# Gadersd/stable-diffusion-burn

Hardware: NVIDIA H100
Metric: images_per_sec_512x512_20steps (higher is better)
Workload: dtype fp16 tensor-core operands (3-term split-fp16 on the two high-res UNet levels), fp32 accumulate

## Files before the change

### include/sdb200.h

```cpp
#ifndef SDB200_H
#define SDB200_H

#include <stddef.h>
#include <stdint.h>

#ifdef __cplusplus
extern "C" {
#endif

typedef struct sdb_ctx sdb_ctx;

int sdb_create(int device, sdb_ctx** out);
int sdb_create_inpaint(int device, sdb_ctx** out);
int sdb_destroy(sdb_ctx* ctx);
const char* sdb_last_error(sdb_ctx* ctx);
const char* sdb_version(void);

int sdb_tensor_count(sdb_ctx* ctx);
int sdb_tensor_info(sdb_ctx* ctx, int index, const char** name, int64_t dims[4], int* ndim);
int sdb_set_tensor(sdb_ctx* ctx, const char* name, const float* host, const int64_t* dims, int ndim);
int sdb_get_tensor(sdb_ctx* ctx, const char* name, float* host, int64_t count);
int sdb_load_dump_dir(sdb_ctx* ctx, const char* path);
int64_t sdb_read_dump_tensor(const char* file, int ndim, int64_t* dims, float* data, int64_t capacity);
int sdb_init_synthetic(sdb_ctx* ctx, uint32_t seed);
// ... 76 lines not shown
int sdb_profile_get(sdb_ctx* ctx, int cls, const char** name, int64_t* launches, double* ms,
                    double* flops, double* bytes);
int sdb_profile_get_issued(sdb_ctx* ctx, int cls, double* issued_flops);
int64_t sdb_launch_count(sdb_ctx* ctx);

int sdb_test_linear(sdb_ctx* ctx, const float* a, const float* w, const float* bias, int M, int K, int N,
                    int passes, float* c);
int sdb_test_gemm_ex(sdb_ctx* ctx, const float* a, const float* w, const float* bias, const float* residual, int M, int K,
                     int N, int passes, int flags, const float* xa, const float* xw, int XK, float* out);
int sdb_test_conv2d(sdb_ctx* ctx, const float* x, const float* w, const float* bias, int n, int cin, int H,
                    int W, int cout, int ksize, int stride, int upsample, int passes, float* y);
int sdb_test_ln_fold(sdb_ctx* ctx, const float* a, const float* a2, const float* w0, const float* b0, const float* gamma,
                     const float* beta, const float* w1, const float* b1, int M, int K0, int C, int N, int passes, int geglu,
                     float* out);
int sdb_test_conv_groupnorm(sdb_ctx* ctx, const float* x, const float* w, const float* bias, const float* gamma,
                            const float* beta, int n, int cin, int H, int W, int cout, int ksize, int stride, int upsample,
                            int passes, int silu, float* y, int* slots);
int sdb_test_groupnorm(sdb_ctx* ctx, const float* x, const float* gamma, const float* beta, int n, int c,
                       int H, int W, int silu, float* y);
int sdb_test_layernorm(sdb_ctx* ctx, const float* x, const float* gamma, const float* beta, int rows, int c,
                       float* y);
int sdb_test_attention(sdb_ctx* ctx, const float* q, const float* k, const float* v, int n, int Nq, int Nk,
                       int C, int heads, const int32_t* kvlen, int flags, float* out);
int sdb_test_resblock(sdb_ctx* ctx, const float* x0, const float* x1, int n, int c0, int c1, int H, int W, int cout,
                      const float* norm1_g, const float* norm1_b, const float* conv1_w, const float* conv1_b, const float* norm2_g,
                      const float* norm2_b, const float* conv2_w, const float* conv2_b, const float* skip_w, const float* skip_b,
                      const float* emb_bias, int passes, int flags, float* out, float* out16, float* out_norm, int32_t* trace);
int sdb_test_groupnorm_cat(sdb_ctx* ctx, const float* x0, const float* x1, int n, int c0, int c1, int H, int W,
                           const float* gamma, const float* beta, int silu, int mode, float* y, int32_t* trace);
int sdb_test_spatial_transformer(sdb_ctx* ctx, int index, const float* x, int n, int c, int H, int W, const float* context,
                                 int lmax, const int32_t* lens, int flags, float* out, float* out16, float* out_norm, float* taps_y,
                                 float* taps_ln, int32_t* trace);
int sdb_test_step_noise(sdb_ctx* ctx, uint64_t noise_seed, int t, int64_t count, float* out);

#ifdef __cplusplus
}
#endif
#endif
```

### stable_diffusion_burn_b200/_lib.py

```python
from __future__ import annotations

import ctypes as C
import os

import numpy as np

_HERE = os.path.dirname(os.path.abspath(__file__))
LIB_PATH = os.path.join(_HERE, "libsdb200.so")

_f32p = C.POINTER(C.c_float)
_u8p = C.POINTER(C.c_uint8)
_i64p = C.POINTER(C.c_int64)
_ctx = C.c_void_p


class SdbBatch(C.Structure):
    _fields_ = [("n", C.c_int), ("L", C.c_int), ("context", C.c_void_p), ("context_len", C.POINTER(C.c_int32)),
                ("Lu", C.c_int), ("uncond", C.c_void_p), ("uncond_len", C.POINTER(C.c_int32)),
                ("guidance_scale", C.POINTER(C.c_double)), ("seed", C.POINTER(C.c_uint64)),
                ("noise_seed", C.POINTER(C.c_uint64))]


_batchp = C.POINTER(SdbBatch)

# ... 46 lines not shown
    ("sdb_lora_remove", C.c_int, [_ctx, C.c_int]),
    ("sdb_lora_apply", C.c_int, [_ctx]),
    ("sdb_get_merged_tensor", C.c_int, [_ctx, C.c_char_p, _f32p, C.c_int64]),
    ("sdb_sample_batch", C.c_int, [_ctx, _batchp, C.c_int, _f32p, C.c_int, C.c_int, _f32p, _u8p]),
    ("sdb_sample_batch_dev", C.c_int, [_ctx, _batchp, C.c_int, C.c_void_p, C.c_int, C.c_int, C.c_void_p, C.c_void_p,
                                       C.c_void_p]),
    ("sdb_img2img_batch", C.c_int, [_ctx, _batchp, _u8p, _u8p, C.c_double, C.c_int, _f32p, C.c_int, C.c_int, _f32p, _u8p]),
    ("sdb_img2img_batch_dev", C.c_int, [_ctx, _batchp, C.c_void_p, C.c_void_p, C.c_double, C.c_int, C.c_void_p, C.c_int,
                                        C.c_int, C.c_void_p, C.c_void_p, C.c_void_p]),
    ("sdb_set_option", C.c_int, [_ctx, C.c_char_p, C.c_int]),
    ("sdb_profile_enable", C.c_int, [_ctx, C.c_int]),
    ("sdb_profile_reset", C.c_int, [_ctx]),
    ("sdb_profile_class_count", C.c_int, [_ctx]),
    ("sdb_profile_get", C.c_int, [_ctx, C.c_int, C.POINTER(C.c_char_p), _i64p, C.POINTER(C.c_double),
                                  C.POINTER(C.c_double), C.POINTER(C.c_double)]),
    ("sdb_profile_get_issued", C.c_int, [_ctx, C.c_int, C.POINTER(C.c_double)]),
    ("sdb_launch_count", C.c_int64, [_ctx]),
    ("sdb_test_linear", C.c_int, [_ctx, _f32p, _f32p, _f32p, C.c_int, C.c_int, C.c_int, C.c_int, _f32p]),
    ("sdb_test_conv2d", C.c_int, [_ctx, _f32p, _f32p, _f32p, C.c_int, C.c_int, C.c_int, C.c_int, C.c_int, C.c_int,
                                  C.c_int, C.c_int, C.c_int, _f32p]),
    ("sdb_test_ln_fold", C.c_int, [_ctx, _f32p, _f32p, _f32p, _f32p, _f32p, _f32p, _f32p, _f32p, C.c_int, C.c_int, C.c_int, C.c_int,
                                   C.c_int, C.c_int, _f32p]),
    ("sdb_test_conv_groupnorm", C.c_int, [_ctx, _f32p, _f32p, _f32p, _f32p, _f32p, C.c_int, C.c_int, C.c_int, C.c_int, C.c_int,
                                          C.c_int, C.c_int, C.c_int, C.c_int, C.c_int, _f32p, C.POINTER(C.c_int)]),
    ("sdb_test_resblock", C.c_int, [_ctx, _f32p, _f32p, C.c_int, C.c_int, C.c_int, C.c_int, C.c_int, C.c_int,
                                    _f32p, _f32p, _f32p, _f32p, _f32p, _f32p, _f32p, _f32p, _f32p, _f32p, _f32p,
                                    C.c_int, C.c_int, _f32p, _f32p, _f32p, C.POINTER(C.c_int32)]),
    ("sdb_test_groupnorm_cat", C.c_int, [_ctx, _f32p, _f32p, C.c_int, C.c_int, C.c_int, C.c_int, C.c_int, _f32p, _f32p,
                                         C.c_int, C.c_int, _f32p, C.POINTER(C.c_int32)]),
    ("sdb_test_spatial_transformer", C.c_int, [_ctx, C.c_int, _f32p, C.c_int, C.c_int, C.c_int, C.c_int, _f32p, C.c_int,
                                               C.POINTER(C.c_int32), C.c_int, _f32p, _f32p, _f32p, _f32p, _f32p,
                                               C.POINTER(C.c_int32)]),
    ("sdb_test_step_noise", C.c_int, [_ctx, C.c_uint64, C.c_int, C.c_int64, _f32p]),
    ("sdb_test_groupnorm", C.c_int, [_ctx, _f32p, _f32p, _f32p, C.c_int, C.c_int, C.c_int, C.c_int, C.c_int, _f32p]),
    ("sdb_test_layernorm", C.c_int, [_ctx, _f32p, _f32p, _f32p, C.c_int, C.c_int, _f32p]),
    ("sdb_test_attention", C.c_int, [_ctx, _f32p, _f32p, _f32p, C.c_int, C.c_int, C.c_int, C.c_int, C.c_int,
                                     C.POINTER(C.c_int32), C.c_int, _f32p]),
]

_lib = None


def load():
    global _lib
    if _lib is None:
        if not os.path.exists(LIB_PATH):
            raise RuntimeError(f"{LIB_PATH} is missing: build it with `python -c 'import __graft_entry__ as g; g.build()'` "
                               "(there is no CPU fallback)")
        lib = C.CDLL(LIB_PATH)
        for name, res, args in SIGNATURES:
            fn = getattr(lib, name)
            fn.restype = res
            fn.argtypes = args
        _lib = lib
    return _lib


def f32(a) -> np.ndarray:
    return np.ascontiguousarray(a, dtype=np.float32)


def ptr(a: np.ndarray):
    return a.ctypes.data_as(_f32p)


class SdbError(RuntimeError):
# ... 436 lines not shown
    def test_groupnorm_cat(self, x0, x1, gamma, beta, silu=False, mode=0):
        x0 = f32(x0)
        n, c0, H, W = x0.shape
        x1 = f32(x1) if x1 is not None else None
        c1 = 0 if x1 is None else x1.shape[1]
        g = f32(gamma); b = f32(beta)
        y = np.empty((n, c0 + c1, H, W), np.float32)
        trace = np.zeros(64, np.int32)
        self.check(self.lib.sdb_test_groupnorm_cat(self.h, ptr(x0), None if x1 is None else ptr(x1), n, c0, c1, H, W, ptr(g), ptr(b),
                                                   1 if silu else 0, int(mode), ptr(y), trace.ctypes.data_as(C.POINTER(C.c_int32))))
        return y, self._decode_trace(trace)

    _EPI_ROLES = ("lns", "lnc", "geglu", "res16", "res32", "gn")

    def test_spatial_transformer(self, index, x, context, lens, act16=True):
        x = f32(x); context = f32(context)
        n, c, H, W = x.shape
        lens = np.ascontiguousarray(lens, dtype=np.int32)
        assert context.shape[0] == n and context.shape[2] == 768 and lens.shape == (n,)
        out, out16, outn = (np.empty((n, c, H, W), np.float32) for _ in range(3))
        y = np.empty((4, n * H * W, c), np.float32)
        ln = np.empty((3, n * H * W, 2), np.float32)
        t = np.zeros(160, np.int32)
        i32 = lambda a: a.ctypes.data_as(C.POINTER(C.c_int32))
        self.check(self.lib.sdb_test_spatial_transformer(self.h, int(index), ptr(x), n, c, H, W, ptr(context), context.shape[1],
                                                         i32(lens), 1 if act16 else 0, ptr(out), ptr(out16), ptr(outn), ptr(y),
                                                         ptr(ln), i32(t)))
        paths = {1: "fused", 2: "apply", 3: "apply+fold"}
        keys = ("kind", "N", "BN", "split", "TN", "TH", "TW", "xk", "gn_slots", "a1", "passes")
        gemms = []
        for i in range(min(int(t[5]), 10)):
            g = dict(zip(keys, (int(v) for v in t[6 + 12 * i:17 + 12 * i])))
            g["epi"] = {r for b, r in enumerate(self._EPI_ROLES) if int(t[17 + 12 * i]) >> b & 1}
            gemms.append(g)
        attn = [dict(zip(("dpad", "Nq", "Nk", "qk3", "kvlen"), (int(v) for v in t[127 + 5 * i:132 + 5 * i])))
                for i in range(min(int(t[126]), 4))]
        tr = {"gn": [paths.get(int(v), int(v)) for v in t[1:1 + min(int(t[0]), 4)]], "gemms": gemms, "attn": attn}
        return dict(out=out, out16=out16, out_norm=outn, y=y, ln=ln, trace=tr)

    def test_groupnorm(self, x, gamma, beta, silu=False):
        x = f32(x); n, c, H, W = x.shape
        y = np.empty_like(x)
        g = f32(gamma); b = f32(beta)
        self.check(self.lib.sdb_test_groupnorm(self.h, ptr(x), ptr(g), ptr(b), n, c, H, W, 1 if silu else 0, ptr(y)))
        return y

    def test_step_noise(self, noise_seed, t, count):
        out = np.empty(int(count), np.float32)
        self.check(self.lib.sdb_test_step_noise(self.h, int(noise_seed), int(t), int(count), ptr(out)))
        return out

    def test_layernorm(self, x, gamma, beta):
        x = f32(x); rows, c = x.shape
        y = np.empty_like(x)
        g = f32(gamma); b = f32(beta)
        self.check(self.lib.sdb_test_layernorm(self.h, ptr(x), ptr(g), ptr(b), rows, c, ptr(y)))
        return y

    def test_attention(self, q, k, v, heads, kvlen=None, causal=False, v_transposed=False):
        q = f32(q); k = f32(k); v = f32(v)
        n, Nq, Cc = q.shape; Nk = k.shape[1]
        out = np.empty_like(q)
        lens = None if kvlen is None else np.ascontiguousarray(kvlen, dtype=np.int32)
        assert lens is None or lens.shape == (n,), "kvlen needs one length per sample"
        flags = (1 if causal else 0) | (2 if v_transposed else 0)
        self.check(self.lib.sdb_test_attention(self.h, ptr(q), ptr(k), ptr(v), n, Nq, Nk, Cc, heads,
# ... 4 lines not shown
```

### stable_diffusion_burn_b200/csrc/api.cu

```cuda
#include "../../include/sdb200.h"

#include <dlfcn.h>

#include <cstdlib>
#include <cstring>
#include <mutex>

#include "attention.cuh"
#include "kernels.cuh"
#include "model.cuh"
#include "runtime.cuh"

using namespace sdb;

struct sdb_ctx {
  Ctx c;
};

static thread_local std::string g_err;

#define API_BEGIN(ctxp)                      \
  if (!(ctxp)) {                             \
    g_err = "null context";                  \
    return 1;                                \
  }                                          \
  Ctx& c = (ctxp)->c;                        \
  try {                                      \
    SDB_CUDA(cudaSetDevice(c.device));

#define API_END                              \
  }                                          \
  catch (const std::exception& e) {          \
    c.err = e.what();                        \
    g_err = c.err;                           \
    return 1;                                \
  }                                          \
  return 0;

static void ctx_teardown(sdb_ctx* h) {
  if (!h) return;
  cudaSetDevice(h->c.device);
// ... 864 lines not shown
                      skip_w, skip_b, emb_bias, passes, flags, out, out16, out_norm, trace);
  API_END
}

int sdb_test_groupnorm_cat(sdb_ctx* ctx, const float* x0, const float* x1, int n, int c0, int c1, int H, int W, const float* gamma,
                           const float* beta, int silu, int mode, float* y, int32_t* trace) {
  API_BEGIN(ctx)
  c.work.reset();
  model_test_groupnorm_cat(c, x0, x1, n, c0, c1, H, W, gamma, beta, silu, mode, y, trace);
  API_END
}

int sdb_test_spatial_transformer(sdb_ctx* ctx, int index, const float* x, int n, int ch, int H, int W, const float* context,
                                 int lmax, const int32_t* lens, int flags, float* out, float* out16, float* out_norm, float* taps_y,
                                 float* taps_ln, int32_t* trace) {
  API_BEGIN(ctx)
  need_final(c);
  c.work.reset();
  model_test_spatial_transformer(c, index, x, n, ch, H, W, context, lmax, lens, flags, out, out16, out_norm, taps_y, taps_ln, trace);
  API_END
}

int sdb_test_step_noise(sdb_ctx* ctx, uint64_t noise_seed, int t, int64_t count, float* out) {
  API_BEGIN(ctx)
  SDB_CHECK(out && count >= 1, "step_noise: null output or count < 1");
  SDB_CHECK(t >= 0 && t < 1000, "step_noise: timestep must be in [0, 1000)");
  float* d = (float*)c.io(0, (size_t)count * 4);
  step_noise_launch(d, (long long)count, noise_seed, t, c.stream);
  SDB_CUDA(cudaMemcpyAsync(out, d, (size_t)count * 4, cudaMemcpyDeviceToHost, c.stream));
  SDB_CUDA(cudaStreamSynchronize(c.stream));
  API_END
}

}
```

### stable_diffusion_burn_b200/csrc/model.cu

```cuda
#include "model.cuh"

#include "../../include/sdb200.h"

#include <algorithm>
#include <cmath>
#include <cstring>
#include <functional>

#include "model_def.cuh"

namespace sdb {

static Model& M(Ctx& c) { return *reinterpret_cast<Model*>(c.model); }
static int round_up(int x, int m) { return (x + m - 1) / m * m; }

static int g_level_passes[4] = {3, 3, 1, 1};
static int g_vae_passes_lowres = 3, g_vae_passes_up = 3, g_vae_passes_highres = 1;

static Half2Ptr alloc_half2(Arena& a, size_t count) {
  Half2Ptr p;
  p.hi = a.get<__half>(count);
  p.lo = a.get<__half>(count);
  return p;
}
// ... 2186 lines not shown
  SpatialTransformerW& st = *m.sts[index];
  SDB_CHECK(Cx == st.c, "test_spatial_transformer: x must have the block's channel count (" + std::to_string(st.c) + ")");
  const int C = st.c, HW = H * W, ls = ln_slots(C);
  const long long Mt = (long long)n * HW;
  Fwd f(c, n);
  f.init_sums(4);
  const int Lpad = round_up(Lmax, 32);
  float* ctxp = c.work.get<float>((size_t)n * Lpad * 768);
  int* d_len = c.work.get<int>(n);
  SDB_CUDA(cudaMemsetAsync(ctxp, 0, (size_t)n * Lpad * 768 * 4, c.stream));
  SDB_CUDA(cudaMemcpy2DAsync(ctxp, (size_t)Lpad * 768 * 4, context, (size_t)Lmax * 768 * 4, (size_t)Lmax * 768 * 4, n,
                             cudaMemcpyHostToDevice, c.stream));
  SDB_CUDA(cudaMemcpyAsync(d_len, lens, 4 * n, cudaMemcpyHostToDevice, c.stream));
  CtxState cs;
  prepare_context(f, ctxp, Lpad, d_len, cs);
  const Act a = stage_activation(f, x, C, H, W, true);
  Act o = (flags & 1) ? f.act16(H, W, C) : f.act(H, W, C);
  StTaps taps;
  for (Half2Ptr& y : taps.y) y = f.half2((size_t)Mt * C, true);
  for (float*& l : taps.ln) l = c.work.get<float>((size_t)Mt * ls * 2);
  ActOp g;
  {
    TraceScope ts(c);
    run_spatial_transformer(f, st, cs, cs.kv[index], a, o, &taps);
    g = f.gn_operand(o, nullptr, st.norm, true, true);
    std::fill(trace, trace + kStTraceInts, 0);
    trace[0] = (int)c.gn_trace.size();
    for (size_t i = 0; i < c.gn_trace.size() && i < 4; ++i) trace[1 + i] = c.gn_trace[i];
    trace[5] = (int)c.gemm_trace.size();
    for (size_t i = 0; i < c.gemm_trace.size() && i < 10; ++i) {
      const Ctx::GemmRecord& r = c.gemm_trace[i];
      const int v[12] = {r.kind, r.N, r.BN, r.split, r.TN, r.TH, r.TW, r.xk_channels, r.gn_slots, r.a1_channels, r.passes, r.epi};
      std::copy(v, v + 12, trace + 6 + 12 * i);
    }
    trace[126] = (int)c.attn_trace.size();
    for (size_t i = 0; i < c.attn_trace.size() && i < 4; ++i) {
      const Ctx::AttnRecord& r = c.attn_trace[i];
      const int v[5] = {r.dpad, r.Nq, r.Nk, r.qk3, r.kvlen};
      std::copy(v, v + 5, trace + 127 + 5 * i);
    }
  }
  float* d = c.work.get<float>(o.count());
  nhwc_to_nchw_launch(o.p, n, C, H, W, d, c.stream);
  SDB_CUDA(cudaMemcpyAsync(out, d, o.count() * 4, cudaMemcpyDeviceToHost, c.stream));
  fetch_half2(c, o.raw16, n, C, H, W, out16);
  fetch_half2(c, g.p, n, C, H, W, out_norm);
  const size_t cnt = (size_t)Mt * C;
  std::vector<__half> hi(cnt), lo(cnt);
  for (int i = 0; i < 4; ++i) {
    SDB_CUDA(cudaMemcpyAsync(hi.data(), taps.y[i].hi, cnt * 2, cudaMemcpyDeviceToHost, c.stream));
    SDB_CUDA(cudaMemcpyAsync(lo.data(), taps.y[i].lo, cnt * 2, cudaMemcpyDeviceToHost, c.stream));
    SDB_CUDA(cudaStreamSynchronize(c.stream));
    for (size_t e = 0; e < cnt; ++e) taps_y[i * cnt + e] = __half2float(hi[e]) + __half2float(lo[e]);
  }
  std::vector<float> sl((size_t)Mt * ls * 2);
  for (int i = 0; i < 3; ++i) {
    SDB_CUDA(cudaMemcpyAsync(sl.data(), taps.ln[i], sl.size() * 4, cudaMemcpyDeviceToHost, c.stream));
    SDB_CUDA(cudaStreamSynchronize(c.stream));
    for (long long r = 0; r < Mt; ++r) {
      float sm = 0.f, sq = 0.f;
      for (int k = 0; k < ls; ++k) sm += sl[(r * ls + k) * 2], sq += sl[(r * ls + k) * 2 + 1];
      taps_ln[(i * Mt + r) * 2] = sm, taps_ln[(i * Mt + r) * 2 + 1] = sq;
    }
  }
}

// ... 2 lines not shown
```

### stable_diffusion_burn_b200/csrc/runtime.cu

```cuda
#include "runtime.cuh"

#include <algorithm>

#include <cudaTypedefs.h>

#include <cmath>
#include <cstdlib>
#include <cstring>

namespace sdb {

int g_pdl_late = 1;
bool g_pdl_enabled = true;
int g_num_sms = 132;

void Arena::init(size_t bytes) {
  SDB_CUDA(cudaMalloc(&base, bytes));
  cap = bytes;
  off = 0;
}
void Arena::destroy() {
  if (base) cudaFree(base);
  base = nullptr;
  cap = off = 0;
}
void* Arena::alloc(size_t bytes) {
  const size_t a = (off + 1023) & ~size_t(1023);
  if (a + bytes > cap)
    throw Error("arena exhausted: need " + std::to_string(a + bytes) + " of " + std::to_string(cap) + " bytes");
  off = a + bytes;
  if (off > high) high = off;
  return base + a;
}
// ... 268 lines not shown
    SDB_CHECK(xk->x0.n == a0.n && xk->x0.H == a0.H && xk->x0.W == a0.W && xk->x0.P == 1 && xk->x0.C % 64 == 0, "extra-K geometry");
    SDB_CHECK(!xk->has_x1 || (xk->x1.n == a0.n && xk->x1.H == a0.H && xk->x1.W == a0.W && xk->x1.C % 64 == 0), "extra-K geometry");
    SDB_CHECK(xk->w.N == w.N && xk->w.K == xC, "extra-K weights");
    SDB_CHECK(passes < 2 || (xk->x0.p.lo && (!xk->has_x1 || xk->x1.p.lo)), "multi-pass GEMM needs the lo half of the extra operands");
    SDB_CHECK(passes < 3 || xk->w.p.lo, "3-pass GEMM needs the lo half of the extra weights");
    p.xkc0 = xk->x0.C / 64, p.xkc = xC / 64;
  }

  p.TW = std::min(pow2_floor(a0.W), 128);
  p.TH = std::min(128 / p.TW, pow2_ceil(a0.H));
  p.TN = 128 / (p.TW * p.TH);
  p.tiles_w = (a0.W + p.TW - 1) / p.TW;
  p.tiles_h = (a0.H + p.TH - 1) / p.TH;
  p.tiles_n = (a0.n + p.TN - 1) / p.TN;
  const int m_tiles = p.tiles_w * p.tiles_h * p.tiles_n;

  int BN;
  if (ep.geglu)
    BN = 128;
  else if (w.N % 160 == 0)
    BN = 160;
  else if (w.N % 256 == 0 && (long long)m_tiles * (w.N / 256) >= 2 * g_num_sms)
    BN = 256;
  else if (w.N % 128 == 0)
    BN = 128;
  else
    BN = 64;
  if (ep.ln_out) {
    SDB_CHECK(w.N % 160 == 0 && !ep.geglu, "LayerNorm statistics need an output width that tiles by 160");
    BN = 160;
  }
  if (ep.ln_in) SDB_CHECK(BN == 128 || BN == 160, "LayerNorm-consuming GEMM: tile width");
  const int n_tiles = (w.N + BN - 1) / BN;


  const int iters = p.num_taps * p.kc + p.xkc;
  int split = 1;
  if (c.opt_splitk && kind != G_CONV3_UP2 && !ep.geglu && !ep.ln_out && !ep.ln_in) {
    const int ctas = m_tiles * n_tiles;
    if (ctas <= g_num_sms / 2 && iters >= c.opt_splitk_min_iters) {
      split = std::min(std::min(g_num_sms / ctas, iters / c.opt_splitk_chunk), 16);
      if (split < 1) split = 1;
    }
  }
  if (split > 1) {
    const int per = (iters + split - 1) / split;
    split = (iters + per - 1) / per;
  }
  p.split_k = split;
  static const bool gemm_dbg = getenv("SDB_GEMM_DBG") != nullptr || getenv("SDB_LABEL_LOG") != nullptr;
  if (c.debug_sync || c.profiling || gemm_dbg) {
    char buf[256];
    snprintf(buf, sizeof(buf), "gemm kind=%d n=%d H=%d W=%d P=%d C0=%d C1=%d N=%d K=%d xk=%d BN=%d split=%d passes=%d geglu=%d epi=%s%s tile=%dx%dx%d",
             kind, a0.n, a0.H, a0.W, a0.P, a0.C, a1in ? a1.C : 0, w.N, w.K, p.xkc * 64, BN, split, passes, ep.geglu,
             ep.gn ? "gn" : (ep.ln_out ? "lns" : (ep.ln_in ? "lnc" : "-")), ep.residual16.hi ? "+r16" : (ep.residual ? "+r32" : ""), p.TN, p.TH, p.TW);
    c.dbg_label = buf;
  }

  GnPart* gn = ep.gn;
  if (gn) {
    int slots = m_tiles / p.tiles_n * split * phases_out;
    bool geom = p.TN <= 4;
    if (kind == G_LINEAR && gn_rpi > 0) {
      const long long rows = (long long)a0.W;
      geom = rows % gn_rpi == 0 && (gn_rpi % 128 == 0 || (128 % gn_rpi == 0 && gn_rpi >= 32));
      gn_nimg = (int)(rows / gn_rpi);
      slots = (gn_rpi >= 128 ? gn_rpi / 128 : 1) * split;
    } else {
      if (kind == G_LINEAR) geom = false;
      gn_rpi = 0;
    }
    const bool ok = gn->buf && gn->bucket > 0 && !ep.geglu && geom && BN >= 128 && BN % gn->bucket == 0 && w.N % gn->bucket == 0 &&
                    slots <= gn->cap && c.opt_gn_epilogue;
    gn->slots = ok ? slots : 0;
    if (!ok) gn = nullptr;
  }
  if (c.trace_on) {
    const int epi = (ep.ln_out ? EPI_ROLE_LNS : 0) | (ep.ln_in ? EPI_ROLE_LNC : 0) | (ep.geglu ? EPI_ROLE_GEGLU : 0) |
                    (ep.residual16.hi ? EPI_ROLE_RES16 : 0) | (ep.residual ? EPI_ROLE_RES32 : 0) | (gn ? EPI_ROLE_GN : 0);
    c.gemm_trace.push_back({kind_in, w.N, BN, split, p.TN, p.TH, p.TW, p.xkc * 64, gn ? gn->slots : 0, a1in ? a1.C : 0, passes, epi});
  }
  p.gn_part = gn ? gn->buf : nullptr;
  p.gn_cap = gn ? gn->cap : 0, p.gn_bucket = gn ? gn->bucket : 1;
  p.gn_rpi = gn ? gn_rpi : 0, p.gn_nimg = gn_nimg;
  p.ln_out = ep.ln_out, p.ln_slots = ln_slots(w.N);
  p.ln_in = ep.ln_in, p.ln_in_slots = ep.ln_in_slots, p.ln_C = ep.ln_C, p.ln_eps = ep.ln_eps;
  p.ln_u = passes >= 3 ? ep.ln_u_full : ep.ln_u_hi;
  SDB_CHECK(!ep.ln_in || (p.ln_u && ep.ln_in_slots > 0 && ep.ln_C == w.K && kind == G_LINEAR), "LayerNorm-consuming GEMM: arguments");
  SDB_CHECK(!ep.ln_in || (!ep.residual && !ep.rowbias && !ep.residual16.hi), "LayerNorm-consuming GEMM: no residual / row bias");
  SDB_CHECK(!ep.ln_out || kind == G_LINEAR, "LayerNorm statistics: rows must be tokens");
  p.res_hi = ep.residual16.hi, p.res_lo = ep.residual16.lo;
  SDB_CHECK(!ep.residual16.hi || (ep.residual16.lo && !ep.residual && !ep.rowbias), "fp16-pair residual: needs both halves, excludes the fp32 residual / row bias");
  p.out_f32 = ep.out_f32;
  p.out_f16 = ep.out_f16.hi;
  p.out_f16_lo = ep.out_f16.lo;
  p.bias = ep.bias;
  p.rowbias = ep.rowbias;
  p.residual = ep.residual;
  p.geglu = ep.geglu;
  p.act = ep.act;
  p.pdl_late = g_pdl_late;
  p.prefetch_w = (g_pdl_enabled && c.opt_prefetch_w && m_tiles <= 4) ? 1 : 0;
  const int nout = ep.geglu ? w.N / 2 : w.N;
  p.ldc = ep.ldc ? ep.ldc : nout;
  p.ldc16 = ep.ldc16 ? ep.ldc16 : nout;
  SDB_CHECK(!(ep.rowbias && ep.residual), "epilogue takes a time-embedding row or a residual, not both");
  p.os = (kind == G_CONV3_UP2) ? 2 : 1;
  p.OH = a0.H * p.os, p.OW = a0.W * p.os;
  SDB_CHECK((double)a0.n * p.OH * p.OW * (double)std::max(p.ldc, p.ldc16) < 2147483648.0,
            "GEMM output exceeds 2^31 elements (the epilogue uses 32-bit element offsets)");

  GemmMaps maps;
  memset(&maps, 0, sizeof(maps));
// ... 36 lines not shown
    maps.b[1] = maps.b[0];
    if (passes >= 3) maps.b[1] = make_w_map(wlo, w.K, wrows, bbox, w.ld);
    maps.bx[0] = maps.bx[1] = maps.b[0];
    if (xk) {
      const int xrows = xk->w.rows ? xk->w.rows : xk->w.N;
      maps.bx[0] = make_w_map(xk->w.p.hi, xk->w.K, xrows, bbox, xk->w.ld);
      maps.bx[1] = passes >= 3 ? make_w_map(xk->w.p.lo, xk->w.K, xrows, bbox, xk->w.ld) : maps.bx[0];
    }
    p.gn_slot0 = 0;
    p.up2 = 0, p.gn_phase_slots = (m_tiles / p.tiles_n) * split;
    if (kind == G_CONV3_UP2) {
      p.up2 = 1, p.oa = 0, p.ob = 0;
      for (int t = 0; t < 4; ++t) p.tap_dh[t] = (t >> 1) - 1, p.tap_dw[t] = (t & 1) - 1, p.tap_ph[t] = 0;
    }
    if (split > 1) {
      const size_t need = (size_t)split * (size_t)Mtot * w.N * sizeof(float);
      p.ws = reinterpret_cast<float*>(c.work.alloc(need));
      SDB_CHECK((long long)m_tiles * n_tiles * 2 <= 65536, "split-K ticket buffer");
      SDB_CHECK((long long)m_tiles * n_tiles * split <= g_num_sms, "split-K CTAs must be co-resident");
      p.tickets = c.splitk_tickets;
    }
    {
      static const bool dbg_on = getenv("SDB_GEMM_DBG") != nullptr;
      static long long* dbg_buf = nullptr;
      if (dbg_on) {
        if (!dbg_buf) SDB_CUDA(cudaMallocManaged(&dbg_buf, 16 * sizeof(long long)));
        SDB_CUDA(cudaStreamSynchronize(c.stream));
        memset(dbg_buf, 0, 16 * sizeof(long long));
        p.dbg = dbg_buf;
      }
      const std::string label = c.dbg_label;
      {
        KernelScope ks(c, KC_GEMM, flops * phases_out, bytes * phases_out, flops * passes * phases_out);
        gemm_tc_launch(maps, p, BN, passes, c.stream);
      }
      if (dbg_on) {
        SDB_CUDA(cudaStreamSynchronize(c.stream));
        fprintf(stderr, "gemm_dbg %s | cycles since entry: prologue %lld tma0 %lld landed %lld lastmma %lld accum %lld epi %lld exit %lld | chunk0: ld %lld stage %lld finish %lld (bias %lld loads0 %lld batch0 %lld)\n",
                label.c_str(), dbg_buf[1] - dbg_buf[0], dbg_buf[2] - dbg_buf[0], dbg_buf[3] - dbg_buf[0],
                dbg_buf[4] - dbg_buf[0], dbg_buf[5] - dbg_buf[0], dbg_buf[6] - dbg_buf[0], dbg_buf[7] - dbg_buf[0], dbg_buf[9] - dbg_buf[8], dbg_buf[10] - dbg_buf[9],
                dbg_buf[11] - dbg_buf[10], dbg_buf[12] - dbg_buf[10], dbg_buf[13] - dbg_buf[12], dbg_buf[14] - dbg_buf[13]);
      }
    }
  }
}

}
```

### stable_diffusion_burn_b200/csrc/runtime.cuh

```cuda
#pragma once
#include <string>
#include <unordered_map>
#include <unordered_set>
#include <vector>

#include "common.cuh"
#include "attention.cuh"
#include "gemm_tc.cuh"
#include "kernels.cuh"

namespace sdb {

struct Arena {
  char* base = nullptr;
  size_t cap = 0, off = 0, high = 0;
  void init(size_t bytes);
  void destroy();
  void* alloc(size_t bytes);
  template <class T>
  T* get(size_t count) {
    return reinterpret_cast<T*>(alloc(count * sizeof(T)));
  }
  void reset() { off = 0; }
};
// ... 95 lines not shown
  std::unordered_map<std::string, float> norm_eps;
  int opt_precision = 0;
  int opt_graphs = 1;
  int opt_splitk = 1;
  int opt_splitk_min_iters = 32, opt_splitk_chunk = 8;
  int opt_skip_merge = 1;
  int opt_raw16 = 1;
  int opt_mlp_passes = 0;
  int opt_attn_split = 1;
  int opt_emb_hoist = 1;
  int opt_prefetch_w = 0;
  int opt_gn_epilogue = 1;
  int sampler_kind = 0;
  double sampler_eta = 0.0;
  uint64_t sampler_noise_seed = 0;
  int unet_cin = 4;
  bool profiling = false;
  std::vector<ProfEvent> prof;
  int64_t launches = 0;
  double cls_ms[KC_COUNT] = {0}, cls_flops[KC_COUNT] = {0}, cls_bytes[KC_COUNT] = {0};
  double cls_issued[KC_COUNT] = {0};
  int64_t cls_launches[KC_COUNT] = {0};
  struct IoBuf {
    void* p = nullptr;
    size_t cap = 0;
  } iobuf[13];
  void* io(int slot, size_t bytes);
  void io_destroy();
  void* model = nullptr;
  unsigned int* splitk_tickets = nullptr;
  bool debug_sync = false;
  std::string dbg_label;
  struct GemmRecord {
    int kind, N, BN, split, TN, TH, TW, xk_channels, gn_slots, a1_channels, passes, epi;
  };
  struct AttnRecord {
    int dpad, Nq, Nk, qk3, kvlen;
  };
  bool trace_on = false;
  std::vector<GemmRecord> gemm_trace;
  std::vector<AttnRecord> attn_trace;
  std::vector<int> gn_trace;

  float* master_ptr(const std::string& name);
  const TensorInfo& info(const std::string& name);
  bool has(const std::string& name) const { return index.count(name) != 0; }
};

struct KernelScope {
  Ctx& c;
  int cls;
  bool on;
  ProfEvent ev;
  KernelScope(Ctx& c, int cls, double flops = 0, double bytes = 0, double issued = 0);
  ~KernelScope();
};
void profile_collect(Ctx& c);

struct ExtraK {
  ActOp x0, x1;
  bool has_x1 = false;
  WeightOp w;
};

void run_gemm(Ctx& c, int kind, const ActOp& a0, const ActOp* a1, const WeightOp& w, int passes, const Epilogue& ep,
              const ExtraK* xk = nullptr);

// ... 23 lines not shown
```

Before: 5.000.

## Add persistent warp-specialized GEGLU GEMM with LayerNorm-consuming epilogue

Adds a persistent TMA+wgmma kernel for the LayerNorm-consuming GEGLU GEMM with 3-pass split-fp16 operands. It is selected when the tile count exceeds the SM count. A producer warp streams A/B chunks through a multi-stage mbarrier ring while two consumer warpgroups alternate tiles, so one group's epilogue overlaps the other's MMA. This is meant to remove wave-quantization and per-tile prologue/epilogue stalls, at the cost of a fixed BN=128 constraint and a new code path that needs its own correctness checks. It also adds a host schedule API and a trace flag for testing.

```diff
diff --git a/include/sdb200.h b/include/sdb200.h
--- a/include/sdb200.h
+++ b/include/sdb200.h
@@ -132,6 +132,7 @@
                                  int lmax, const int32_t* lens, int flags, float* out, float* out16, float* out_norm, float* taps_y,
                                  float* taps_ln, int32_t* trace);
 int sdb_test_step_noise(sdb_ctx* ctx, uint64_t noise_seed, int t, int64_t count, float* out);
+int sdb_gemm_lnc_schedule(int ntiles, int kchunks, int num_sms, int stages, int32_t* out);
 
 #ifdef __cplusplus
 }
diff --git a/stable_diffusion_burn_b200/_lib.py b/stable_diffusion_burn_b200/_lib.py
--- a/stable_diffusion_burn_b200/_lib.py
+++ b/stable_diffusion_burn_b200/_lib.py
@@ -102,6 +102,7 @@
                                                C.POINTER(C.c_int32), C.c_int, _f32p, _f32p, _f32p, _f32p, _f32p,
                                                C.POINTER(C.c_int32)]),
     ("sdb_test_step_noise", C.c_int, [_ctx, C.c_uint64, C.c_int, C.c_int64, _f32p]),
+    ("sdb_gemm_lnc_schedule", C.c_int, [C.c_int, C.c_int, C.c_int, C.c_int, C.POINTER(C.c_int32)]),
     ("sdb_test_groupnorm", C.c_int, [_ctx, _f32p, _f32p, _f32p, C.c_int, C.c_int, C.c_int, C.c_int, C.c_int, _f32p]),
     ("sdb_test_layernorm", C.c_int, [_ctx, _f32p, _f32p, _f32p, C.c_int, C.c_int, _f32p]),
     ("sdb_test_attention", C.c_int, [_ctx, _f32p, _f32p, _f32p, C.c_int, C.c_int, C.c_int, C.c_int, C.c_int,
@@ -604,6 +605,7 @@
         for i in range(min(int(t[5]), 10)):
             g = dict(zip(keys, (int(v) for v in t[6 + 12 * i:17 + 12 * i])))
             g["epi"] = {r for b, r in enumerate(self._EPI_ROLES) if int(t[17 + 12 * i]) >> b & 1}
+            g["persistent"] = bool(int(t[147]) >> i & 1)
             gemms.append(g)
         attn = [dict(zip(("dpad", "Nq", "Nk", "qk3", "kvlen"), (int(v) for v in t[127 + 5 * i:132 + 5 * i])))
                 for i in range(min(int(t[126]), 4))]
diff --git a/stable_diffusion_burn_b200/csrc/api.cu b/stable_diffusion_burn_b200/csrc/api.cu
--- a/stable_diffusion_burn_b200/csrc/api.cu
+++ b/stable_diffusion_burn_b200/csrc/api.cu
@@ -2,11 +2,13 @@
 
 #include <dlfcn.h>
 
+#include <algorithm>
 #include <cstdlib>
 #include <cstring>
 #include <mutex>
 
 #include "attention.cuh"
+#include "gemm_lnc.cuh"
 #include "kernels.cuh"
 #include "model.cuh"
 #include "runtime.cuh"
@@ -937,4 +939,18 @@
   API_END
 }
 
-}
+int sdb_gemm_lnc_schedule(int ntiles, int kchunks, int num_sms, int stages, int32_t* out) {
+  if (ntiles < 1 || kchunks < 1 || num_sms < 1 || stages < 1 || !out) return -1;
+  const int grid = std::min(ntiles, num_sms);
+  for (int cta = 0; cta < grid; ++cta) {
+    const int nseq = sdb::lnc_cta_tiles(ntiles, cta, grid) * kchunks;
+    for (int seq = 0; seq < nseq; ++seq, out += 7) {
+      const sdb::LncChunk c = sdb::lnc_chunk(seq, kchunks, cta, grid, stages);
+      const int32_t rec[7] = {cta, seq, c.tile, c.k, c.stage, (int32_t)c.phase, c.consumer};
+      std::copy(rec, rec + 7, out);
+    }
+  }
+  return 0;
+}
+
+}
diff --git a/stable_diffusion_burn_b200/csrc/gemm_lnc.cu b/stable_diffusion_burn_b200/csrc/gemm_lnc.cu
--- /dev/null
+++ b/stable_diffusion_burn_b200/csrc/gemm_lnc.cu
@@ -0,0 +1,237 @@
+#include "gemm_lnc.cuh"
+
+#include <algorithm>
+
+namespace sdb {
+
+namespace {
+
+constexpr int BM = 128;
+constexpr int BK = 64;
+constexpr int A_TILE_BYTES = BM * BK * 2;
+constexpr int SMEM_OPTIN_MAX = 227 * 1024;
+
+template <int BN>
+struct LncStage {
+  static constexpr int B_TILE_BYTES = BN * BK * 2;
+  static constexpr int BYTES = 2 * A_TILE_BYTES + 2 * B_TILE_BYTES;
+};
+template <int BN>
+__host__ __device__ constexpr int lnc_stages() {
+  constexpr int n = (SMEM_OPTIN_MAX - 1024) / (LncStage<BN>::BYTES + 2 * 8);
+  return n > 8 ? 8 : n;
+}
+
+__device__ __forceinline__ void store_pair16(float y0, float y1, unsigned int o16, __half* out_f16, __half* out_f16_lo) {
+  const __half2 h = f2h2_sat(y0, y1);
+  *reinterpret_cast<__half2*>(out_f16 + o16) = h;
+  if (out_f16_lo) {
+    const float2 f = __half22float2(h);
+    *reinterpret_cast<__half2*>(out_f16_lo + o16) = __floats2half2_rn(y0 - f.x, y1 - f.y);
+  }
+}
+
+template <int BN>
+__global__ void __launch_bounds__(384, 1)
+gemm_lnc_persistent_kernel(const __grid_constant__ GemmMaps maps, const GemmParams p, int n_tiles, int ntiles) {
+  using L = LncStage<BN>;
+  constexpr int STAGES = lnc_stages<BN>();
+  extern __shared__ __align__(1024) uint8_t smem_raw[];
+  uint8_t* smem = smem_raw + ((1024u - (smem_u32(smem_raw) & 1023u)) & 1023u);
+  uint64_t* full_bar = reinterpret_cast<uint64_t*>(smem + STAGES * L::BYTES);
+  uint64_t* empty_bar = full_bar + STAGES;
+
+  const int warp = threadIdx.x >> 5;
+  const int lane = threadIdx.x & 31;
+  const int kc = p.kc;
+  const int my_tiles = lnc_cta_tiles(ntiles, blockIdx.x, gridDim.x);
+  const int nseq = my_tiles * kc;
+  long long* const dbg = (p.dbg && blockIdx.x == 0) ? p.dbg : nullptr;
+  if (dbg && threadIdx.x == 0) dbg[0] = clock64();
+  if (!p.pdl_late) pdl_trigger();
+
+  if (threadIdx.x == 0) {
+    for (int s = 0; s < STAGES; ++s) {
+      mbar_init(&full_bar[s], 1);
+      mbar_init(&empty_bar[s], 4);
+    }
+    fence_mbar_init();
+  }
+  if (warp == 0 && lane == 0) {
+    tma_prefetch_desc(&maps.a[0][0]);
+    tma_prefetch_desc(&maps.b[0]);
+  }
+  __syncthreads();
+  if (dbg && threadIdx.x == 0) dbg[1] = clock64();
+
+  if (warp < 4) {
+    asm volatile("setmaxnreg.dec.sync.aligned.u32 40;");
+    if (warp == 0 && elect_one()) {
+      auto load_b = [&](const LncChunk& c) {
+        uint8_t* sb = smem + c.stage * L::BYTES + 2 * A_TILE_BYTES;
+        const int col0 = (c.tile % n_tiles) * BN;
+        tma_load_2d(sb, &maps.b[0], &full_bar[c.stage], c.k * BK, col0);
+        tma_load_2d(sb + L::B_TILE_BYTES, &maps.b[1], &full_bar[c.stage], c.k * BK, col0);
+      };
+      auto load_a = [&](const LncChunk& c) {
+        uint8_t* st = smem + c.stage * L::BYTES;
+        const int w0 = (c.tile / n_tiles) * BM;
+        tma_load_5d(st, &maps.a[0][0], &full_bar[c.stage], c.k * BK, w0, 0, 0, 0);
+        tma_load_5d(st + A_TILE_BYTES, &maps.a[0][1], &full_bar[c.stage], c.k * BK, w0, 0, 0, 0);
+      };
+      const int npre = min(STAGES, nseq);
+      for (int seq = 0; seq < npre; ++seq) {
+        const LncChunk c = lnc_chunk(seq, kc, blockIdx.x, gridDim.x, STAGES);
+        mbar_expect_tx(&full_bar[c.stage], L::BYTES);
+        load_b(c);
+      }
+      pdl_wait();
+      for (int seq = 0; seq < npre; ++seq) load_a(lnc_chunk(seq, kc, blockIdx.x, gridDim.x, STAGES));
+      if (dbg) dbg[2] = clock64();
+      for (int seq = npre; seq < nseq; ++seq) {
+        const LncChunk c = lnc_chunk(seq, kc, blockIdx.x, gridDim.x, STAGES);
+        mbar_wait(&empty_bar[c.stage], c.phase ^ 1u);
+        mbar_expect_tx(&full_bar[c.stage], L::BYTES);
+        load_a(c);
+        load_b(c);
+      }
+    }
+  } else {
+    asm volatile("setmaxnreg.inc.sync.aligned.u32 232;");
+    pdl_wait();
+    const int g = (warp - 4) >> 2;
+    const int wq = warp & 3;
+    const bool stamp = dbg && wq == 0 && lane == 0;
+    const int cq = 2 * (lane & 3);
+    for (int i = g; i < my_tiles; i += 2) {
+      const int tile = blockIdx.x + i * gridDim.x;
+      const int mt = tile / n_tiles, nt = tile - mt * n_tiles;
+      const bool last = i == my_tiles - 1;
+      float acc[2][BN / 2];
+#pragma unroll
+      for (int h = 0; h < 2; ++h)
+#pragma unroll
+        for (int j = 0; j < BN / 2; ++j) acc[h][j] = 0.f;
+      int prev = -1;
+      if (i > 0) asm volatile("bar.sync %0, 256;" ::"r"(1 + g) : "memory");
+      for (int k = 0; k < kc; ++k) {
+        const LncChunk c = lnc_chunk(i * kc + k, kc, blockIdx.x, gridDim.x, STAGES);
+        mbar_wait(&full_bar[c.stage], c.phase);
+        if (dbg && threadIdx.x == 128 && i == 0 && k == 0) dbg[3] = clock64();
+        const uint32_t a_hi = smem_u32(smem + c.stage * L::BYTES);
+        const uint32_t a_lo = a_hi + A_TILE_BYTES;
+        const uint32_t b_hi = a_hi + 2 * A_TILE_BYTES;
+        const uint32_t b_lo = b_hi + L::B_TILE_BYTES;
+        wgmma_fence();
+#pragma unroll
+        for (int kk = 0; kk < BK / 16; ++kk) {
+          const uint32_t koff = kk * 32;
+          const uint64_t db = make_sdesc_sw128(b_hi + koff), db_lo = make_sdesc_sw128(b_lo + koff);
+#pragma unroll
+          for (int h = 0; h < 2; ++h) {
+            const uint64_t da = make_sdesc_sw128(a_hi + h * (64 * 128) + koff);
+            Wgmma<BN>::template ss<0>(acc[h], da, db, 1);
+            Wgmma<BN>::template ss<0>(acc[h], make_sdesc_sw128(a_lo + h * (64 * 128) + koff), db, 1);
+            Wgmma<BN>::template ss<0>(acc[h], da, db_lo, 1);
+          }
+        }
+        wgmma_commit();
+        wgmma_wait<1>();
+        if (prev >= 0 && lane == 0) mbar_arrive(&empty_bar[prev]);
+        prev = c.stage;
+      }
+      if (i + 1 < my_tiles) asm volatile("bar.arrive %0, 256;" ::"r"(2 - g) : "memory");
+      wgmma_wait<0>();
+      reg_fence(acc[0]);
+      reg_fence(acc[1]);
+      if (lane == 0) mbar_arrive(&empty_bar[prev]);
+      if (stamp && last) dbg[4] = clock64();
+      if (last && p.pdl_late) pdl_trigger();
+
+      const int row0 = mt * BM;
+      float ln_mu = 0.f, ln_rs = 0.f;
+      {
+        const int r = row0 + 64 * (lane >> 4) + 16 * wq + (lane & 15);
+        if (r < p.W) {
+          const float2* sp = reinterpret_cast<const float2*>(p.ln_in) + (size_t)r * p.ln_in_slots;
+          float sm = 0.f, sq = 0.f;
+          for (int s = 0; s < p.ln_in_slots; ++s) {
+            const float2 v = sp[s];
+            sm += v.x, sq += v.y;
+          }
+          const float inv = 1.0f / (float)p.ln_C;
+          ln_mu = sm * inv;
+          ln_rs = rsqrtf(fmaxf(sq * inv - ln_mu * ln_mu, 0.f) + p.ln_eps);
+        }
+      }
+      int mr[2][2];
+      float rmu[2][2], rrs[2][2];
+#pragma unroll
+      for (int h = 0; h < 2; ++h)
+#pragma unroll
+        for (int s = 0; s < 2; ++s) {
+          const int src = 16 * h + 8 * s + (lane >> 2);
+          const int r = row0 + 64 * h + 16 * wq + 8 * s + (lane >> 2);
+          mr[h][s] = r < p.W ? r : -1;
+          rmu[h][s] = __shfl_sync(0xffffffffu, ln_mu, src);
+          rrs[h][s] = __shfl_sync(0xffffffffu, ln_rs, src);
+        }
+      if (stamp && last) dbg[5] = clock64();
+      constexpr int HB = BN / 2;
+      const int col0 = nt * BN, ocol0 = nt * HB;
+#pragma unroll
+      for (int jj = 0; jj < HB / 8; ++jj) {
+        const int c = 8 * jj + cq;
+        const float2 bx = *reinterpret_cast<const float2*>(p.bias + col0 + c);
+        const float2 bg = *reinterpret_cast<const float2*>(p.bias + col0 + HB + c);
+        const float2 ux = *reinterpret_cast<const float2*>(p.ln_u + col0 + c);
+        const float2 ug = *reinterpret_cast<const float2*>(p.ln_u + col0 + HB + c);
+#pragma unroll
+        for (int h = 0; h < 2; ++h)
+#pragma unroll
+          for (int s = 0; s < 2; ++s) {
+            if (mr[h][s] < 0) continue;
+            const int j = 4 * jj + 2 * s;
+            float tx0 = acc[h][j], tx1 = acc[h][j + 1], tg0 = acc[h][j + HB / 2], tg1 = acc[h][j + 1 + HB / 2];
+            const float m = rmu[h][s], r = rrs[h][s];
+            tx0 = r * (tx0 - m * ux.x), tx1 = r * (tx1 - m * ux.y);
+            tg0 = r * (tg0 - m * ug.x), tg1 = r * (tg1 - m * ug.y);
+            const float y0 = (tx0 + bx.x) * gelu_erf_fast(tg0 + bg.x);
+            const float y1 = (tx1 + bx.y) * gelu_erf_fast(tg1 + bg.y);
+            store_pair16(y0, y1, (unsigned)(mr[h][s] * p.ldc16 + ocol0 + c), p.out_f16, p.out_f16_lo);
+          }
+      }
+      if (stamp && last) dbg[6] = clock64();
+    }
+  }
+  __syncthreads();
+  if (dbg && threadIdx.x == 0) dbg[7] = clock64();
+}
+
+template <int BN>
+void launch(const GemmMaps& maps, const GemmParams& p, int n_tiles, int ntiles, cudaStream_t stream) {
+  constexpr int smem = lnc_stages<BN>() * LncStage<BN>::BYTES + 2 * lnc_stages<BN>() * 8 + 1024;
+  static_assert(smem <= SMEM_OPTIN_MAX, "shared memory per block");
+  static DeviceOnce once;
+  if (once.first())
+    SDB_CUDA(cudaFuncSetAttribute(gemm_lnc_persistent_kernel<BN>, cudaFuncAttributeMaxDynamicSharedMemorySize, smem));
+  launch_k(gemm_lnc_persistent_kernel<BN>, dim3(std::min(ntiles, g_num_sms)), dim3(384), (size_t)smem, stream, maps, p,
+           n_tiles, ntiles);
+}
+
+}
+
+void gemm_lnc_persistent_launch(const GemmMaps& maps, const GemmParams& p, int BN, cudaStream_t stream) {
+  SDB_CHECK(p.TN == 1 && p.TH == 1 && p.TW == BM && p.nimg == 1 && p.H == 1, "persistent LayerNorm GEMM: rows must be tokens");
+  SDB_CHECK(p.num_taps == 1 && p.kc0 == p.kc && p.xkc == 0 && p.split_k == 1 && !p.up2, "persistent LayerNorm GEMM: K loop");
+  SDB_CHECK(p.geglu && p.bias && p.ln_in && p.ln_u && p.out_f16 && !p.out_f32 && !p.gn_part && !p.ln_out && !p.residual &&
+                !p.rowbias && !p.res_hi,
+            "persistent LayerNorm GEMM: epilogue");
+  SDB_CHECK(BN == 128 && p.N % BN == 0, "persistent LayerNorm GEMM: tile width");
+  const int n_tiles = p.N / BN;
+  const long long ntiles = (long long)p.tiles_w * n_tiles;
+  SDB_CHECK(ntiles < (1ll << 31) / 16, "persistent LayerNorm GEMM: tile count");
+  launch<128>(maps, p, n_tiles, (int)ntiles, stream);
+}
+
+}
diff --git a/stable_diffusion_burn_b200/csrc/gemm_lnc.cuh b/stable_diffusion_burn_b200/csrc/gemm_lnc.cuh
--- /dev/null
+++ b/stable_diffusion_burn_b200/csrc/gemm_lnc.cuh
@@ -0,0 +1,29 @@
+#pragma once
+#include "gemm_tc.cuh"
+
+namespace sdb {
+
+struct LncChunk {
+  int tile, k, stage, consumer;
+  unsigned int phase;
+};
+__host__ __device__ inline int lnc_cta_tiles(int ntiles, int cta, int grid) {
+  return cta < ntiles ? (ntiles - cta + grid - 1) / grid : 0;
+}
+__host__ __device__ inline LncChunk lnc_chunk(int seq, int kchunks, int cta, int grid, int stages) {
+  const int i = seq / kchunks;
+  LncChunk c;
+  c.tile = cta + i * grid;
+  c.k = seq - i * kchunks;
+  c.stage = seq % stages;
+  c.phase = (unsigned int)((seq / stages) & 1);
+  c.consumer = i & 1;
+  return c;
+}
+
+inline bool gemm_lnc_persistent_selected(bool ln_in, bool geglu, int passes, long long tiles, int num_sms) {
+  return ln_in && geglu && passes == 3 && tiles > num_sms;
+}
+void gemm_lnc_persistent_launch(const GemmMaps& maps, const GemmParams& p, int BN, cudaStream_t stream);
+
+}
diff --git a/stable_diffusion_burn_b200/csrc/model.cu b/stable_diffusion_burn_b200/csrc/model.cu
--- a/stable_diffusion_burn_b200/csrc/model.cu
+++ b/stable_diffusion_burn_b200/csrc/model.cu
@@ -2242,6 +2242,7 @@
       const Ctx::GemmRecord& r = c.gemm_trace[i];
       const int v[12] = {r.kind, r.N, r.BN, r.split, r.TN, r.TH, r.TW, r.xk_channels, r.gn_slots, r.a1_channels, r.passes, r.epi};
       std::copy(v, v + 12, trace + 6 + 12 * i);
+      trace[147] |= r.persistent << i;
     }
     trace[126] = (int)c.attn_trace.size();
     for (size_t i = 0; i < c.attn_trace.size() && i < 4; ++i) {
diff --git a/stable_diffusion_burn_b200/csrc/runtime.cu b/stable_diffusion_burn_b200/csrc/runtime.cu
--- a/stable_diffusion_burn_b200/csrc/runtime.cu
+++ b/stable_diffusion_burn_b200/csrc/runtime.cu
@@ -1,4 +1,6 @@
 #include "runtime.cuh"
+
+#include "gemm_lnc.cuh"
 
 #include <algorithm>
 
@@ -333,6 +335,8 @@
   }
   if (ep.ln_in) SDB_CHECK(BN == 128 || BN == 160, "LayerNorm-consuming GEMM: tile width");
   const int n_tiles = (w.N + BN - 1) / BN;
+  const bool lnc_persistent =
+      gemm_lnc_persistent_selected(ep.ln_in != nullptr, ep.geglu != 0, passes, (long long)m_tiles * n_tiles, g_num_sms);
 
 
   const int iters = p.num_taps * p.kc + p.xkc;
@@ -352,9 +356,10 @@
   static const bool gemm_dbg = getenv("SDB_GEMM_DBG") != nullptr || getenv("SDB_LABEL_LOG") != nullptr;
   if (c.debug_sync || c.profiling || gemm_dbg) {
     char buf[256];
-    snprintf(buf, sizeof(buf), "gemm kind=%d n=%d H=%d W=%d P=%d C0=%d C1=%d N=%d K=%d xk=%d BN=%d split=%d passes=%d geglu=%d epi=%s%s tile=%dx%dx%d",
+    snprintf(buf, sizeof(buf), "gemm kind=%d n=%d H=%d W=%d P=%d C0=%d C1=%d N=%d K=%d xk=%d BN=%d split=%d passes=%d geglu=%d epi=%s%s tile=%dx%dx%d%s",
              kind, a0.n, a0.H, a0.W, a0.P, a0.C, a1in ? a1.C : 0, w.N, w.K, p.xkc * 64, BN, split, passes, ep.geglu,
-             ep.gn ? "gn" : (ep.ln_out ? "lns" : (ep.ln_in ? "lnc" : "-")), ep.residual16.hi ? "+r16" : (ep.residual ? "+r32" : ""), p.TN, p.TH, p.TW);
+             ep.gn ? "gn" : (ep.ln_out ? "lns" : (ep.ln_in ? "lnc" : "-")), ep.residual16.hi ? "+r16" : (ep.residual ? "+r32" : ""), p.TN, p.TH, p.TW,
+             lnc_persistent ? " persistent" : "");
     c.dbg_label = buf;
   }
 
@@ -379,7 +384,8 @@
   if (c.trace_on) {
     const int epi = (ep.ln_out ? EPI_ROLE_LNS : 0) | (ep.ln_in ? EPI_ROLE_LNC : 0) | (ep.geglu ? EPI_ROLE_GEGLU : 0) |
                     (ep.residual16.hi ? EPI_ROLE_RES16 : 0) | (ep.residual ? EPI_ROLE_RES32 : 0) | (gn ? EPI_ROLE_GN : 0);
-    c.gemm_trace.push_back({kind_in, w.N, BN, split, p.TN, p.TH, p.TW, p.xkc * 64, gn ? gn->slots : 0, a1in ? a1.C : 0, passes, epi});
+    c.gemm_trace.push_back({kind_in, w.N, BN, split, p.TN, p.TH, p.TW, p.xkc * 64, gn ? gn->slots : 0, a1in ? a1.C : 0, passes, epi,
+                            lnc_persistent ? 1 : 0});
   }
   p.gn_part = gn ? gn->buf : nullptr;
   p.gn_cap = gn ? gn->cap : 0, p.gn_bucket = gn ? gn->bucket : 1;
@@ -482,7 +488,10 @@
       const std::string label = c.dbg_label;
       {
         KernelScope ks(c, KC_GEMM, flops * phases_out, bytes * phases_out, flops * passes * phases_out);
-        gemm_tc_launch(maps, p, BN, passes, c.stream);
+        if (lnc_persistent)
+          gemm_lnc_persistent_launch(maps, p, BN, c.stream);
+        else
+          gemm_tc_launch(maps, p, BN, passes, c.stream);
       }
       if (dbg_on) {
         SDB_CUDA(cudaStreamSynchronize(c.stream));
diff --git a/stable_diffusion_burn_b200/csrc/runtime.cuh b/stable_diffusion_burn_b200/csrc/runtime.cuh
--- a/stable_diffusion_burn_b200/csrc/runtime.cuh
+++ b/stable_diffusion_burn_b200/csrc/runtime.cuh
@@ -151,7 +151,7 @@
   bool debug_sync = false;
   std::string dbg_label;
   struct GemmRecord {
-    int kind, N, BN, split, TN, TH, TW, xk_channels, gn_slots, a1_channels, passes, epi;
+    int kind, N, BN, split, TN, TH, TW, xk_channels, gn_slots, a1_channels, passes, epi, persistent;
   };
   struct AttnRecord {
     int dpad, Nq, Nk, qk3, kvlen;
```

After: 5.022, median of 6. Within noise of the previous version (+0.4%).
